# PimDeWitte/pde-engine

Hardware: AMD Instinct MI355X
Metric: validated candidates/sec (force-free depth-4 batch, 64x64 grid + p*) (higher is better)
Workload: dtype f64; 1 GPU; force_free validated candidates (force_free_d4_validated.npz, 142004 programs) tiled+shuffled(seed 0) to 2097152/GPU; 64x64 grid + ref point; problem=force_free, candidates_per_gpu=2097152, points_per_candidate=4097, full_grid=True, parallelism=shard1

## Files before the change

pde-engine_amd/csrc/pdeval.hip:

```cpp
#include <dlfcn.h>
#include <hip/hip_runtime.h>
#include <rccl/rccl.h>

#include <algorithm>
#include <cmath>
#include <cstdlib>
#include <cstdio>
#include <cstring>
#include <map>
#include <string>
#include <vector>

#include "../../include/pdeval.h"
#include "pdeval_kernels.h"
#include "pdeval_point.h"
#include "pdeval_tier2.h"
#include "pdeval_launch.h"
#include "pdeval_foliation.h"

using namespace pd;

#define PD_VERSION "pdeval 0.2 gfx950"

enum {
    L_DEFER = 0,
    L_CPLX = 1,
    L_DEFER2 = 2,
    L_ESC = 3,
    L_ESC_DEEP = 4,
    L_ESC_C = 5,
    L_CPLX_DEEP = 6,
    L_ESC_DEEP2 = 7,
    L_PDEEP = 8,
    L_DD = 9,
    L_DDC = 10,
    L_DD8 = 11,
    L_ESC_C_DEEP = 12,
    L_SLOW = 13,
    L_SLOW2 = 14,
    L_SLOW_C = 15,
    L_DDL = 16,
    L_DDLC = 17,
    L_DDL8 = 18,
    PD_N_LISTS = 19
};
enum { Q_PASS2 = 0, Q_CPLX, Q_T2, Q_T2_3, Q_T2_8, Q_T2_C, Q_T2_C8, Q_N };
#ifndef PD_LIST_QUEUE
#define PD_LIST_QUEUE 0
#endif
#ifndef PD_LIST_PARTS
#define PD_LIST_PARTS 1
#endif
constexpr int PD_COUNT_WORDS = PD_N_LISTS + 1 + Q_N;

namespace {
struct Grid {
    double x_lo, x_hi, nx, y_lo, y_hi, ny, x_ph, y_ph;
};
}

struct pdeval_ctx {
    int device = 0;
    int problem = 0;
    int n_ref = 0, n_pts = 0;
    int fp_pts[PDEVAL_FP_N] = {0, 0, 0, 0};
    hipStream_t stream = nullptr;
    hipStream_t side = nullptr;
    hipEvent_t ev_fork = nullptr, ev_join = nullptr;
    bool dd_early = true;
    int list_queue = PD_LIST_QUEUE;
    int list_parts = PD_LIST_PARTS;
    uint8_t* d_ddps = nullptr;
    double* d_dd_res = nullptr;
    double* d_dd_q = nullptr;
    bool dd_spec = true;
    double ref_x[4] = {0, 0, 0, 0}, ref_y[4] = {0, 0, 0, 0};
    dd ref_xd[4] = {}, ref_yd[4] = {};
    dd kc_ref[16] = {};
    int nx = 0, ny = 0;
    double* d_gx = nullptr;
    double* d_gy = nullptr;
    double* d_kc = nullptr;
    double* d_ptab = nullptr;
    Grid grid{};
    bool grid_default = true;
    pdeval_kerr_constants kconst{};
    PrmTab<double> prm_pt{}, prm_grid{};
    PrmTab<dd> prm_pt_dd{}, prm_grid_dd{};
    double ct_x[8] = {}, ct_y[8] = {};
    int n_ct = 0;
    int64_t cap = 0;
    int64_t* d_list[PD_N_LISTS] = {};
    int32_t* d_counts = nullptr;
    uint8_t* d_pstate = nullptr;
    int32_t* d_dec = nullptr;
    int64_t dec_cap = 0;
    bool hoist = true;
    bool hoist_sub = true;
    double* d_hoist = nullptr;
    uint32_t* d_hoist_own = nullptr;
    bool hoist_slots = true;
    int32_t* d_hseg = nullptr;
// ... 262 lines not shown
    }
    c->nx = nx;
    c->ny = ny;
    c->n_pts = c->n_ref + nx * ny;
    const int G = nx * ny;
    c->fp_pts[0] = 0;
    for (int f = 1; f < PDEVAL_FP_N; ++f) c->fp_pts[f] = c->n_ref + (int)((int64_t)G * f / PDEVAL_FP_N) + 7 % G;
    auto fail = [&](const char* what, hipError_t e) {
        g_err = std::string(what) + ": " + hipGetErrorString(e);
        pdeval_destroy(c);
        return PDEVAL_ERR_HIP;
    };
    hipError_t e;
    if ((e = hipSetDevice(device_id)) != hipSuccess) return fail("hipSetDevice", e);
    if (const char* v = getenv("PDEVAL_SORT")) c->sort = atoi(v) != 0;
    if (const char* v = getenv("PDEVAL_LEAN_CPLX")) c->lean_cplx = atoi(v) != 0;
    if (const char* v = getenv("PDEVAL_GRAPH")) c->use_graph = atoi(v) != 0;
    if (const char* v = getenv("PDEVAL_DD_EARLY")) c->dd_early = atoi(v) != 0;
    if (const char* v = getenv("PDEVAL_DD_SPEC")) c->dd_spec = atoi(v) != 0;
    if (const char* v = getenv("PDEVAL_LIST_QUEUE")) c->list_queue = std::max(0, atoi(v));
    if (const char* v = getenv("PDEVAL_LIST_PARTS")) c->list_parts = std::min(16, std::max(1, atoi(v)));
    if (const char* v = getenv("PDEVAL_HOIST")) c->hoist = atoi(v) != 0;
    if (const char* v = getenv("PDEVAL_HOIST_SUB")) c->hoist_sub = atoi(v) != 0;
    if (const char* v = getenv("PDEVAL_HOIST_SLOTS")) c->hoist_slots = atoi(v) != 0;
    if (const char* v = getenv("PDEVAL_TIER2_MASK")) c->tier2_mask = atoi(v) != 0;
    if (const char* v = getenv("PDEVAL_DEEP_PARTS")) c->deep_parts = atoi(v) > 1 ? PD_DEEP_PARTS : 1;
    if ((e = hipStreamCreateWithFlags(&c->stream, hipStreamNonBlocking)) != hipSuccess)
        return fail("hipStreamCreate", e);
    if ((e = hipStreamCreateWithFlags(&c->side, hipStreamNonBlocking)) != hipSuccess)
        return fail("hipStreamCreate", e);
    if ((e = hipEventCreateWithFlags(&c->ev_fork, hipEventDisableTiming)) != hipSuccess ||
        (e = hipEventCreateWithFlags(&c->ev_join, hipEventDisableTiming)) != hipSuccess)
        return fail("hipEventCreate", e);
    if ((e = hipMalloc(&c->d_gx, 2 * nx * sizeof(double))) != hipSuccess) return fail("hipMalloc", e);
    if ((e = hipMalloc(&c->d_gy, ny * sizeof(double))) != hipSuccess) return fail("hipMalloc", e);
    if (problem_id == PDEVAL_PROBLEM_KERR &&
        (e = hipMalloc(&c->d_kc, 8 * (size_t)c->n_pts * sizeof(double))) != hipSuccess)
        return fail("hipMalloc", e);
    if (problem_id == PDEVAL_PROBLEM_KERR) pdeval_default_kerr_constants(&c->kconst);
    if (int rc = build_points(c)) {
        g_err = c->err;
        pdeval_destroy(c);
        return rc;
    }
    if ((e = hipMalloc(&c->d_counts, PD_COUNT_WORDS * sizeof(int32_t))) != hipSuccess) return fail("hipMalloc", e);
    *out = c;
    return PDEVAL_OK;
}

extern "C" int pdeval_destroy(pdeval_ctx* c) {
    if (!c) return PDEVAL_ERR_ARG;
    (void)hipSetDevice(c->device);
    if (c->stream) (void)hipStreamSynchronize(c->stream);
    if (c->side) (void)hipStreamSynchronize(c->side);
    if (c->comm) pdeval_comm_destroy(c);
    for (int64_t* l : c->d_list)
        if (l) (void)hipFree(l);
    if (c->d_pstate) (void)hipFree(c->d_pstate);
    if (c->d_ddps) (void)hipFree(c->d_ddps);
    if (c->d_dd_res) (void)hipFree(c->d_dd_res);
    if (c->d_dd_q) (void)hipFree(c->d_dd_q);
    if (c->d_dec) (void)hipFree(c->d_dec);
    if (c->d_hoist) (void)hipFree(c->d_hoist);
    if (c->d_hoist_own) (void)hipFree(c->d_hoist_own);
    if (c->d_hseg) (void)hipFree(c->d_hseg);
    if (c->d_fmask) (void)hipFree(c->d_fmask);
    if (c->d_fsum) (void)hipFree(c->d_fsum);
    if (c->d_status) (void)hipFree(c->d_status);
    if (c->d_noise) (void)hipFree(c->d_noise);
    if (c->d_t2acc) (void)hipFree(c->d_t2acc);
    if (c->d_skeys) (void)hipFree(c->d_skeys);
    if (c->d_sidx) (void)hipFree(c->d_sidx);
    if (c->d_stemp) (void)hipFree(c->d_stemp);
    for (void* p : {(void*)c->d_gx, (void*)c->d_gy, (void*)c->d_kc, (void*)c->d_ptab,
                    (void*)c->d_counts, (void*)c->d_ops, (void*)c->d_off, (void*)c->d_outbuf})
        if (p) (void)hipFree(p);
    for (auto& g : c->graphs)
        if (g.second.exec) (void)hipGraphExecDestroy(g.second.exec);
    if (c->h_stage) (void)hipHostFree(c->h_stage);
    if (c->h_errw) (void)hipHostFree(c->h_errw);
    for (hipEvent_t& e : c->ev)
        if (e) (void)hipEventDestroy(e);
    if (c->ev_fork) (void)hipEventDestroy(c->ev_fork);
    if (c->ev_join) (void)hipEventDestroy(c->ev_join);
    if (c->side) (void)hipStreamDestroy(c->side);
    if (c->stream) (void)hipStreamDestroy(c->stream);
    delete c;
    return PDEVAL_OK;
}

extern "C" const char* pdeval_last_error(pdeval_ctx* c) { return c ? c->err.c_str() : g_err.c_str(); }
extern "C" int pdeval_n_ref_points(pdeval_ctx* c) { return c ? c->n_ref : -1; }
extern "C" int pdeval_n_points(pdeval_ctx* c) { return c ? c->n_pts : -1; }
extern "C" const char* pdeval_version(void) { return PD_VERSION; }

extern "C" int pdeval_default_params(int problem_id, pdeval_params* p) {
    if (!p) return PDEVAL_ERR_ARG;
    p->tau_point = 1e-10;
    p->tau_grid = 1e-7;
    p->kerr_abs_tol = 1e-10;
    p->full_grid = 1;
    p->max_bad = 0;
    p->strict_symbolic = 1;
    p->reserved = 0;
    p->noise_kappa = 16.0;
    p->point_abs_tol = 1e-20;
    p->res_rel_acc = 1e-11;
    p->omega2 = 0.0;
    p->omega2_lo = 0.0;
    (void)problem_id;
    return PDEVAL_OK;
}

static int op_has_imm(uint32_t op) {
    return op == PDOP_PUSH_C || op == PDOP_ADDC || op == PDOP_MULC || op == PDOP_RDIVC || op == PDOP_POW;
}
static int op_words(int32_t w) {
// ... 234 lines not shown
    if (c->d_hseg) (void)hipFree(c->d_hseg);
    c->d_hseg = nullptr;
    if (c->hoist) {
        const int K = c->problem == PDEVAL_PROBLEM_FORCE_FREE ? 4 : 2;
        if (c->hoist_slots && !c->d_hoist) {
            HIPCHK(c, hipMalloc(&c->d_hoist, (size_t)8 * pd::kHoistPool * pd::hoist_stride(K) * sizeof(double)));
            HIPCHK(c, hipMalloc(&c->d_hoist_own, (size_t)8 * pd::kHoistPool * sizeof(uint32_t)));
            HIPCHK(c, hipMemset(c->d_hoist_own, 0, (size_t)8 * pd::kHoistPool * sizeof(uint32_t)));
        } else if (!c->hoist_slots) {
            if (c->d_hoist) (void)hipFree(c->d_hoist);
            c->d_hoist = nullptr;
            HIPCHK(c, hipMalloc(&c->d_hoist, (size_t)std::max<int64_t>(cap, 8 * pd::kHoistPool) * pd::hoist_stride(K) * sizeof(double)));
        }
        HIPCHK(c, hipMalloc(&c->d_hseg, (size_t)cap * 4 * sizeof(int32_t)));
    }
    if (c->d_fmask) (void)hipFree(c->d_fmask);
    c->d_fmask = nullptr;
    if (c->d_fsum) (void)hipFree(c->d_fsum);
    c->d_fsum = nullptr;
    if (c->tier2_mask) {
        HIPCHK(c, hipMalloc(&c->d_fmask, (size_t)cap * c->nx * (c->ny / 64) * sizeof(uint64_t)));
        HIPCHK(c, hipMalloc(&c->d_fsum, (size_t)cap * sizeof(uint64_t)));
    }
    if (c->d_status) (void)hipFree(c->d_status);
    c->d_status = nullptr;
    HIPCHK(c, hipMalloc(&c->d_status, cap));
    if (c->d_noise) (void)hipFree(c->d_noise);
    c->d_noise = nullptr;
    HIPCHK(c, hipMalloc(&c->d_noise, cap * 4 * sizeof(double)));
    if (c->d_t2acc) (void)hipFree(c->d_t2acc);
    c->d_t2acc = nullptr;
    HIPCHK(c, hipMalloc(&c->d_t2acc, cap * sizeof(T2Acc)));
    HIPCHK(c, hipMemset(c->d_t2acc, 0, cap * sizeof(T2Acc)));
    if (c->d_skeys) (void)hipFree(c->d_skeys);
    if (c->d_sidx) (void)hipFree(c->d_sidx);
    if (c->d_stemp) (void)hipFree(c->d_stemp);
    c->d_skeys = nullptr;
    c->d_sidx = nullptr;
    c->d_stemp = nullptr;
    HIPCHK(c, hipMalloc(&c->d_skeys, 2 * cap * sizeof(uint64_t)));
    HIPCHK(c, hipMalloc(&c->d_sidx, 2 * cap * sizeof(int32_t)));
    c->stemp_bytes = sort_temp_bytes(cap);
    HIPCHK(c, hipMalloc(&c->d_stemp, c->stemp_bytes ? c->stemp_bytes : 16));
    c->cap = cap;
    return PDEVAL_OK;
}

template <class T, int K, int MAXD> constexpr size_t stack_lds(int waves) {
    return (size_t)waves * (MAXD - 1) * ((K + 1) * (K + 2) / 2) * 64 * sizeof(T);
}

#ifndef PD_T2_PARTS
#define PD_T2_PARTS 4
#endif
#ifndef PD_T2_PARTS_C
#define PD_T2_PARTS_C 16
#endif
template <class T, int K, int MAXD> constexpr size_t tier2_lds() {
    return (size_t)(MAXD - 1) * ((K + 1) * (K + 2) / 2) * 64 * (sizeof(T) + sizeof(double));
}

#ifndef PD_DD_EARLY_MIN_N
#define PD_DD_EARLY_MIN_N 1024
#endif

__global__ __launch_bounds__(256) void sanitize_list_kernel(const int64_t* list, int32_t* count, int64_t cap,
// ... 118 lines not shown
        KernelArgs b = follow(L_PDEEP, -1, L_ESC);
        launch_point_list(PROB, 0, lgrid, s, b);
        HIPCHK(c, hipGetLastError());
    }
    if constexpr (FF) {
        KernelArgs b = follow(L_CPLX, -1, L_ESC_C);
        launch_point_list(PROB, 1, lgrid, s, b);
        HIPCHK(c, hipGetLastError());
    }
    auto dd_lists = [&](int l0, int lc, int l8) {
        KernelArgs b = a;
        b.defer_list = c->d_list[l0];
        b.defer_count = cnt + l0;
        b.cplx_list = c->d_list[lc];
        b.cplx_count = cnt + lc;
        b.esc_list = c->d_list[l8];
        b.esc_count = cnt + l8;
        return b;
    };
    const unsigned cgrid = (unsigned)((n + 255) / 256);
    const bool early = c->dd_early && n >= PD_DD_EARLY_MIN_N;
    a.dd_spec = early && c->dd_spec ? 1 : 0;
    if (early) {
        hipLaunchKernelGGL((dd_collect_kernel<PROB, DD_EARLY>), dim3(cgrid), dim3(256), 0, s, dd_lists(L_DD, L_DDC, L_DD8));
        HIPCHK(c, hipGetLastError());
        HIPCHK(c, hipEventRecord(c->ev_fork, s));
        HIPCHK(c, hipStreamWaitEvent(c->side, c->ev_fork, 0));
        launch_dd_point(PROB, 0, lgrid, c->side, follow(L_DD, -1, L_ESC), true);
        if (dmax > 2) launch_dd_point(PROB, 1, lgrid, c->side, follow(L_DD8, -1, L_ESC), true);
        if constexpr (FF) launch_dd_point(PROB, 2, lgrid, c->side, follow(L_DDC, -1, L_ESC), true);
        HIPCHK(c, hipGetLastError());
        HIPCHK(c, hipEventRecord(c->ev_join, c->side));
    }
    mark(2);
    launch_decode(PROB, n, s, a);
    HIPCHK(c, hipGetLastError());
    launch_grid(PROB, n, s, a, c->d_list[L_SLOW], cnt + L_SLOW);
    HIPCHK(c, hipGetLastError());
    hipLaunchKernelGGL((validate_kernel<PROB, double, 2, true>), dim3((unsigned)std::min<int64_t>(blocks, 256)),
                       dim3(64), (stack_lds<double, K, 2>(1)), s, follow(L_SLOW, L_DEFER, L_ESC));
    HIPCHK(c, hipGetLastError());
    mark(3);
    if (dmax > 2) {
        hipLaunchKernelGGL(sanitize_list_kernel, dim3(64), dim3(256), 0, s, c->d_list[L_DEFER], cnt + L_DEFER, c->cap, n,
                           a.errw, (uint32_t)ERRW_GRID_LIST);
        launch_grid_list(PROB, pgrid, s, queue(follow(L_DEFER, L_DEFER2, L_ESC), Q_PASS2), c->d_list[L_SLOW2],
                         cnt + L_SLOW2, lparts);
        HIPCHK(c, hipGetLastError());
        hipLaunchKernelGGL((validate_kernel<PROB, double, 3, true>), dim3((unsigned)std::min<int64_t>(blocks, 256)),
                           dim3(64), (stack_lds<double, K, 3>(1)), s, follow(L_SLOW2, L_DEFER2, L_ESC));
        HIPCHK(c, hipGetLastError());
    }
    mark(4);
    if (dmax > 3) {
        if (c->deep_parts > 1)
            hipLaunchKernelGGL((validate_kernel<PROB, double, PDEVAL_MAX_STACK, true, PD_DEEP_PARTS>),
                               dim3((unsigned)std::min<int64_t>(4 * blocks, 1024)), dim3(64),
                               (stack_lds<double, K, PDEVAL_MAX_STACK>(1)), s, follow(L_DEFER2, -1, L_ESC));
        else
            hipLaunchKernelGGL((validate_kernel<PROB, double, PDEVAL_MAX_STACK, true>),
                               dim3((unsigned)std::min<int64_t>(4 * blocks, 1024)), dim3(64),
                               (stack_lds<double, K, PDEVAL_MAX_STACK>(1)), s, follow(L_DEFER2, -1, L_ESC));
        HIPCHK(c, hipGetLastError());
    }
    if constexpr (FF) {
        mark(5);
        if (c->lean_cplx) {
            hipLaunchKernelGGL(sanitize_list_kernel, dim3(64), dim3(256), 0, s, c->d_list[L_CPLX], cnt + L_CPLX, c->cap,
                               n, a.errw, (uint32_t)ERRW_CPLX);
            launch_grid_cplx(pgrid, s, queue(follow(L_CPLX, L_CPLX_DEEP, L_ESC_C), Q_CPLX), c->d_list[L_SLOW_C],
                             cnt + L_SLOW_C, lparts);
            HIPCHK(c, hipGetLastError());
            hipLaunchKernelGGL((validate_kernel<PROB, cplx, 2, true>), dim3((unsigned)std::min<int64_t>(blocks, 256)),
                               dim3(64), (stack_lds<cplx, K, 2>(1)), s, follow(L_SLOW_C, L_CPLX_DEEP, L_ESC_C));
        } else {
            hipLaunchKernelGGL((validate_kernel<PROB, cplx, 2, true>), dim3(pgrid), dim3(64),
                               (stack_lds<cplx, K, 2>(1)), s, follow(L_CPLX, L_CPLX_DEEP, L_ESC_C));
        }
        HIPCHK(c, hipGetLastError());
        mark(6);
        if (dmax > 2) {
            if (c->deep_parts > 1)
                hipLaunchKernelGGL((validate_kernel<PROB, cplx, PDEVAL_MAX_STACK, true, PD_DEEP_PARTS>),
                                   dim3((unsigned)std::min<int64_t>(4 * blocks, 512)), dim3(64),
                                   (stack_lds<cplx, K, PDEVAL_MAX_STACK>(1)), s, follow(L_CPLX_DEEP, -1, L_ESC_C));
            else
                hipLaunchKernelGGL((validate_kernel<PROB, cplx, PDEVAL_MAX_STACK, true>),
                                   dim3((unsigned)std::min<int64_t>(4 * blocks, 512)), dim3(64),
                                   (stack_lds<cplx, K, PDEVAL_MAX_STACK>(1)), s, follow(L_CPLX_DEEP, -1, L_ESC_C));
            HIPCHK(c, hipGetLastError());
        }
    } else {
        mark(5);
        mark(6);
    }
    KernelArgs t = queue(follow(L_ESC, L_ESC_DEEP, L_ESC), Q_T2);
    mark(7);
    hipLaunchKernelGGL((tier2_kernel<PROB, double, 2, false, PD_T2_PARTS>), dim3((unsigned)std::min<int64_t>(n * PD_T2_PARTS, 8192)),
                       dim3(64), (tier2_lds<double, K, 2>()), s, t);
    HIPCHK(c, hipGetLastError());
    mark(8);
    if (dmax > 2) {
        hipLaunchKernelGGL((tier2_kernel<PROB, double, 3, false, PD_T2_PARTS>), dim3((unsigned)std::min<int64_t>(n * PD_T2_PARTS, 4096)),
                           dim3(64), (tier2_lds<double, K, 3>()), s, queue(follow(L_ESC_DEEP, L_ESC_DEEP2, L_ESC), Q_T2_3));
        HIPCHK(c, hipGetLastError());
    }
    mark(9);
    if (dmax > 3) {
        hipLaunchKernelGGL((tier2_kernel<PROB, double, PDEVAL_MAX_STACK>), dim3((unsigned)std::min<int64_t>(n, 512)),
                           dim3(64), (tier2_lds<double, K, PDEVAL_MAX_STACK>()), s, queue(follow(L_ESC_DEEP2, -1, L_ESC), Q_T2_8));
        HIPCHK(c, hipGetLastError());
    }
    if constexpr (FF) {
        mark(10);
        hipLaunchKernelGGL((tier2_kernel<PROB, cplx, 4, false, PD_T2_PARTS_C>),
                           dim3((unsigned)std::min<int64_t>(n * PD_T2_PARTS_C, 4096)), dim3(64),
                           (tier2_lds<cplx, K, 4>()), s, queue(follow(L_ESC_C, L_ESC_C_DEEP, L_ESC_C), Q_T2_C));
        HIPCHK(c, hipGetLastError());
        if (dmax > 4) {
            hipLaunchKernelGGL((tier2_kernel<PROB, cplx, PDEVAL_MAX_STACK, true>), dim3((unsigned)std::min<int64_t>(n, 256)),
                               dim3(64), 0, s, queue(follow(L_ESC_C_DEEP, -1, L_ESC_C), Q_T2_C8));
            HIPCHK(c, hipGetLastError());
        }
    } else {
        mark(10);
    }
    mark(11);
    if (early) {
        HIPCHK(c, hipStreamWaitEvent(s, c->ev_join, 0));
        hipLaunchKernelGGL((dd_collect_kernel<PROB, DD_LATE>), dim3(cgrid), dim3(256), 0, s, dd_lists(L_DDL, L_DDLC, L_DDL8));
        HIPCHK(c, hipGetLastError());
        launch_dd_point(PROB, 0, lgrid, s, follow(L_DDL, -1, L_ESC));
        if (dmax > 2) launch_dd_point(PROB, 1, lgrid, s, follow(L_DDL8, -1, L_ESC));
        if constexpr (FF) launch_dd_point(PROB, 2, lgrid, s, follow(L_DDLC, -1, L_ESC));
        HIPCHK(c, hipGetLastError());
        launch_dd_apply(PROB, (unsigned)std::min<int64_t>(cgrid, 1024), s, dd_lists(L_DD, L_DDC, L_DD8));
        HIPCHK(c, hipGetLastError());
    } else {
        hipLaunchKernelGGL((dd_collect_kernel<PROB, DD_ALL>), dim3(cgrid), dim3(256), 0, s, dd_lists(L_DD, L_DDC, L_DD8));
        HIPCHK(c, hipGetLastError());
        launch_dd_point(PROB, 0, lgrid, s, follow(L_DD, -1, L_ESC));
        if (dmax > 2) launch_dd_point(PROB, 1, lgrid, s, follow(L_DD8, -1, L_ESC));
        if constexpr (FF) launch_dd_point(PROB, 2, lgrid, s, follow(L_DDC, -1, L_ESC));
        HIPCHK(c, hipGetLastError());
    }
    mark(PDEVAL_N_PASSES);
    c->ev_recorded = c->timing ? 1 : 0;
    return PDEVAL_OK;
}

static int check_errw(pdeval_ctx* c, uint32_t w, const char* path, int64_t n, int captured);

static int validate_device(pdeval_ctx* c, const int32_t* d_ops, int64_t n_words, const int64_t* d_offsets,
                           int64_t n, const pdeval_params* params, const pdeval_outputs* d_out, void* stream,
                           int zero_bits, int dmax) {
    if (!c || !d_out || n < 0 || (n > 0 && (!d_ops || !d_offsets)) || n_words < 0) {
        if (c) c->err = "pdeval_validate_device: bad argument";
        return PDEVAL_ERR_ARG;
// ... 69 lines not shown
        d->q_grid = (double*)p; p += 8 * n;
        d->res_ref = (double*)p; p += 8 * n * c->n_ref;
        d->fingerprint = (double*)p; p += 8 * n * PDEVAL_FP_N;
        d->n_bad = (int32_t*)p; p += 4 * n;
        d->n_nonfinite = (int32_t*)p;
    }
    return need;
}

static int validate_small(pdeval_ctx* c, const int32_t* ops, int64_t n_words, const int64_t* offsets, int64_t n,
                          const pdeval_params* params, pdeval_outputs* out, int dmax) {
    if (n_words > kSmallWords) return kGraphFallback;
    if (c->hcap_words < kSmallWords || c->hcap_n < PD_GRAPH_MAX_N + 1) {
        ++c->buf_epoch;
        const int64_t w = std::max<int64_t>(kSmallWords, c->hcap_words);
        const int64_t m = std::max<int64_t>(PD_GRAPH_MAX_N + 1, c->hcap_n);
        if (c->d_ops) (void)hipFree(c->d_ops);
        if (c->d_off) (void)hipFree(c->d_off);
        c->d_ops = nullptr;
        c->d_off = nullptr;
        c->hcap_words = c->hcap_n = 0;
        HIPCHK(c, hipMalloc(&c->d_ops, w * sizeof(int32_t)));
        HIPCHK(c, hipMalloc(&c->d_off, m * sizeof(int64_t)));
        c->hcap_words = w;
        c->hcap_n = m;
    }
    const int64_t need_max = outbuf_layout(c, PD_GRAPH_MAX_N, nullptr);
    if (c->outbuf_bytes < need_max) {
        ++c->buf_epoch;
        if (c->d_outbuf) (void)hipFree(c->d_outbuf);
        c->d_outbuf = nullptr;
        c->outbuf_bytes = 0;
        HIPCHK(c, hipMalloc(&c->d_outbuf, need_max));
        c->outbuf_bytes = need_max;
    }
    int rc = ensure_scratch(c, n);
    if (rc) return rc;
    rc = ensure_dec(c, c->hcap_words);
    if (rc) return rc;
    const size_t in_bytes = kSmallWords * 4 + (PD_GRAPH_MAX_N + 1) * 8;
    if (!c->h_stage) {
        HIPCHK(c, hipHostMalloc((void**)&c->h_stage, in_bytes + need_max + 16, hipHostMallocDefault));
        c->h_stage_bytes = in_bytes + need_max + 16;
    }
    pdeval_params prm;
    if (params) prm = *params;
    else pdeval_default_params(c->problem, &prm);
    dmax = dmax <= 2 ? 2 : dmax <= 4 ? dmax : PDEVAL_MAX_STACK;
    uint64_t key = 1469598103934665603ull;
    auto mix = [&](const void* p, size_t len) {
        const uint8_t* b = (const uint8_t*)p;
        for (size_t i = 0; i < len; ++i) key = (key ^ b[i]) * 1099511628211ull;
    };
    mix(&n, sizeof(n));
    mix(&dmax, sizeof(dmax));
    mix(&prm, sizeof(prm));
    pdeval_outputs d{};
    const int64_t need = outbuf_layout(c, n, &d);
    hipStream_t s = c->stream;
    auto it = c->graphs.find(key);
    if (it != c->graphs.end() && it->second.epoch != c->buf_epoch) {
        (void)hipGraphExecDestroy(it->second.exec);
        c->graphs.erase(it);
        it = c->graphs.end();
    }
    int fresh = 0;
// ... 80 lines not shown
        }
        dmax = std::max(dmax, d);
    }
    HIPCHK(c, hipSetDevice(c->device));
    if (n <= PD_GRAPH_MAX_N && c->use_graph && !c->timing) {
        const int rc = validate_small(c, ops, n_words, offsets, n, params, out, dmax);
        if (rc != kGraphFallback) return rc;
    }
    if (n_words > c->hcap_words) {
        ++c->buf_epoch;
        if (c->d_ops) (void)hipFree(c->d_ops);
        c->d_ops = nullptr;
        c->hcap_words = 0;
        HIPCHK(c, hipMalloc(&c->d_ops, n_words * sizeof(int32_t)));
        c->hcap_words = n_words;
    }
    if (n + 1 > c->hcap_n) {
        ++c->buf_epoch;
        if (c->d_off) (void)hipFree(c->d_off);
        c->d_off = nullptr;
        c->hcap_n = 0;
        HIPCHK(c, hipMalloc(&c->d_off, (n + 1) * sizeof(int64_t)));
        c->hcap_n = n + 1;
    }
    const int64_t nb = ((n + 31) / 32) * 4;
    const int64_t sz_bits = (nb + 15) / 16 * 16, sz_st = (n + 15) / 16 * 16;
    const int64_t need = sz_bits + sz_st + 8 * n * (3 + c->n_ref + PDEVAL_FP_N) + 8 * n * 2;
    if (need > c->outbuf_bytes) {
        ++c->buf_epoch;
        if (c->d_outbuf) (void)hipFree(c->d_outbuf);
        c->d_outbuf = nullptr;
        c->outbuf_bytes = 0;
        HIPCHK(c, hipMalloc(&c->d_outbuf, need));
        c->outbuf_bytes = need;
    }
    uint8_t* p = c->d_outbuf;
    pdeval_outputs d{};
    d.verdict_bits = p; p += sz_bits;
    d.status = p; p += sz_st;
    d.q_ref = (double*)p; p += 8 * n;
    d.q_grid = (double*)p; p += 8 * n;
    d.res_ref = (double*)p; p += 8 * n * c->n_ref;
    d.fingerprint = (double*)p; p += 8 * n * PDEVAL_FP_N;
    d.n_bad = (int32_t*)p; p += 4 * n;
    d.n_nonfinite = (int32_t*)p; p += 4 * n;
    hipStream_t s = c->stream;
    HIPCHK(c, hipMemcpyAsync(c->d_ops, ops, n_words * sizeof(int32_t), hipMemcpyHostToDevice, s));
    HIPCHK(c, hipMemcpyAsync(c->d_off, offsets, (n + 1) * sizeof(int64_t), hipMemcpyHostToDevice, s));
    int rc = validate_device(c, c->d_ops, n_words, c->d_off, n, params, &d, s, 1, dmax);
    if (rc) return rc;
    auto dl = [&](void* h, const void* dv, size_t bytes) -> int {
        if (h) HIPCHK(c, hipMemcpyAsync(h, dv, bytes, hipMemcpyDeviceToHost, s));
        return PDEVAL_OK;
    };
    if ((rc = dl(out->verdict_bits, d.verdict_bits, (n + 7) / 8))) return rc;
    if ((rc = dl(out->status, d.status, n))) return rc;
    if ((rc = dl(out->q_ref, d.q_ref, 8 * n))) return rc;
    if ((rc = dl(out->q_grid, d.q_grid, 8 * n))) return rc;
    if ((rc = dl(out->res_ref, d.res_ref, 8 * n * c->n_ref))) return rc;
    if ((rc = dl(out->fingerprint, d.fingerprint, 8 * n * PDEVAL_FP_N))) return rc;
    if ((rc = dl(out->n_bad, d.n_bad, 4 * n))) return rc;
    if ((rc = dl(out->n_nonfinite, d.n_nonfinite, 4 * n))) return rc;
    uint32_t* herr = reinterpret_cast<uint32_t*>(c->h_errw);
    if (!herr) {
        HIPCHK(c, hipHostMalloc((void**)&c->h_errw, 16, hipHostMallocDefault));
        herr = reinterpret_cast<uint32_t*>(c->h_errw);
// ... 5 lines not shown

extern "C" int pdeval_set_timing(pdeval_ctx* c, int enable) {
    if (!c) return PDEVAL_ERR_ARG;
    HIPCHK(c, hipSetDevice(c->device));
    if (enable && !c->ev[0])
        for (hipEvent_t& e : c->ev) HIPCHK(c, hipEventCreate(&e));
    c->timing = enable != 0;
    c->ev_recorded = 0;
    return PDEVAL_OK;
}

extern "C" int pdeval_pass_times(pdeval_ctx* c, float* ms, int max_passes, const char** names) {
    if (!c || !ms || max_passes < 0) return PDEVAL_ERR_ARG;
    if (!c->ev_recorded) {
        c->err = "pdeval_pass_times: no timed call (pdeval_set_timing(ctx, 1) first)";
        return PDEVAL_ERR_ARG;
    }
    HIPCHK(c, hipSetDevice(c->device));
    HIPCHK(c, hipEventSynchronize(c->ev[PDEVAL_N_PASSES]));
    const int n = max_passes < PDEVAL_N_PASSES ? max_passes : PDEVAL_N_PASSES;
    for (int k = 0; k < n; ++k) {
        HIPCHK(c, hipEventElapsedTime(&ms[k], c->ev[k], c->ev[k + 1]));
        if (names) names[k] = kPassNames[k];
    }
    return PDEVAL_OK;
}

extern "C" int pdeval_pass_counts(pdeval_ctx* c, int64_t* counts, int max_counts) {
    if (!c || !counts || max_counts < 0) return PDEVAL_ERR_ARG;
    HIPCHK(c, hipSetDevice(c->device));
    int32_t h[PD_N_LISTS] = {0};
    HIPCHK(c, hipDeviceSynchronize());
    HIPCHK(c, hipMemcpy(h, c->d_counts, sizeof(h), hipMemcpyDeviceToHost));
    for (int k = 0; k < max_counts && k < PD_N_LISTS; ++k) counts[k] = h[k];
    return PDEVAL_OK;
}

extern "C" int pdeval_eval_points(pdeval_ctx* c, const int32_t* prog, int64_t n_words, const double* xs,
                                  const double* ys, int n_pts, int tier2, double* out, double* jets) {
    if (!c || !prog || !xs || !ys || !out || n_pts <= 0 || n_pts > (1 << 20)) return PDEVAL_ERR_ARG;
    const int d = pdeval_program_depth(prog, n_words);
    if (d < 0 || d > PDEVAL_MAX_STACK) {
        c->err = "pdeval_eval_points: malformed program";
        return PDEVAL_ERR_PROGRAM;
    }
    if (c->problem == PDEVAL_PROBLEM_KERR) {
        c->err = "pdeval_eval_points: force-free only";
        return PDEVAL_ERR_ARG;
    }
    HIPCHK(c, hipSetDevice(c->device));
    int32_t* d_prog = nullptr;
    double *d_x = nullptr, *d_y = nullptr, *d_out = nullptr, *d_jets = nullptr;
    const size_t jet_bytes = (size_t)n_pts * 2 * 15 * sizeof(double);
    auto cleanup = [&]() {
        for (void* q : {(void*)d_prog, (void*)d_x, (void*)d_y, (void*)d_out, (void*)d_jets})
            if (q) (void)hipFree(q);
    };
    hipError_t e = hipSuccess;
    if ((e = hipMalloc(&d_prog, n_words * 4)) == hipSuccess && (e = hipMalloc(&d_x, n_pts * 8)) == hipSuccess &&
        (e = hipMalloc(&d_y, n_pts * 8)) == hipSuccess && (e = hipMalloc(&d_out, n_pts * 32)) == hipSuccess &&
        (e = hipMemcpy(d_prog, prog, n_words * 4, hipMemcpyHostToDevice)) == hipSuccess &&
        (e = hipMemcpy(d_x, xs, n_pts * 8, hipMemcpyHostToDevice)) == hipSuccess &&
        (e = hipMemcpy(d_y, ys, n_pts * 8, hipMemcpyHostToDevice)) == hipSuccess &&
        (!jets || (e = hipMalloc(&d_jets, jet_bytes)) == hipSuccess)) {
        constexpr int K = 4, MAXD = PDEVAL_MAX_STACK;
        hipLaunchKernelGGL((eval_points_kernel<PDEVAL_PROBLEM_FORCE_FREE, MAXD>), dim3((n_pts + 63) / 64), dim3(64),
// ... 153 lines not shown
```

pde-engine_amd/csrc/pdeval_grid.h:

```cpp
#pragma once

#include "pdeval_kernels.h"

namespace pd {

#ifndef PD_LEAN_RSLOT
#define PD_LEAN_RSLOT 1
#endif

constexpr uint64_t op_bit(int op) { return 1ull << op; }
constexpr int PTAB_N = 17;
constexpr uint64_t kImmMask = op_bit(PDOP_PUSH_C) | op_bit(PDOP_ADDC) | op_bit(PDOP_MULC) |
                              op_bit(PDOP_RDIVC) | op_bit(PDOP_POW);
constexpr uint64_t kPushMask = op_bit(PDOP_PUSH_X) | op_bit(PDOP_PUSH_Y) | op_bit(PDOP_PUSH_C) |
                               op_bit(PDOP_PUSH_P);
constexpr uint64_t kBinMask = op_bit(PDOP_ADD) | op_bit(PDOP_SUB) | op_bit(PDOP_RSUB) |
                              op_bit(PDOP_MUL) | op_bit(PDOP_DIV) | op_bit(PDOP_RDIV);
constexpr uint64_t kUnaryMask =
    op_bit(PDOP_ADDC) | op_bit(PDOP_MULC) | op_bit(PDOP_RDIVC) | op_bit(PDOP_NEG) |
    op_bit(PDOP_ADD_X) | op_bit(PDOP_ADD_Y) | op_bit(PDOP_SUB_X) | op_bit(PDOP_SUB_Y) |
    op_bit(PDOP_MUL_X) | op_bit(PDOP_MUL_Y) | op_bit(PDOP_DIV_X) | op_bit(PDOP_DIV_Y) |
    op_bit(PDOP_POWN) | op_bit(PDOP_POW) | op_bit(PDOP_EXP) | op_bit(PDOP_LOG) | op_bit(PDOP_ABS) |
    op_bit(PDOP_SQRT) | op_bit(PDOP_ADD_P) | op_bit(PDOP_SUB_P) | op_bit(PDOP_MUL_P) |
    op_bit(PDOP_DIV_P) | op_bit(PDOP_RDIV_P);
// ... 243 lines not shown
        last = pc;
        pc += len;
    }
    ok = ok && d == 1 && last >= 0;
    if (ok) dec[last] |= (int32_t)(1u << 20);
    uint32_t hp = 0u;
    if (PD_HOIST && ok && hoist_last >= 0 && hoist_heavy) {
        const uint32_t at = (uint32_t)hoist_last + (((uint32_t)dec[hoist_last] >> DEC_DIST) & DEC_DIST_MAX);
        if (at < (uint32_t)plen && at < (1u << 14)) hp = at;
    }
    dec[0] = ok ? (int32_t)(((uint32_t)dmax << 8) | (sg[1] < 0 ? 1u << 16 : 0u) | (hp << 17) |
                            (hp && hoist_y ? 1u << 31 : 0u)) : (int32_t)0xff;
    if (a.hseg) {
        int best = -1;
        const bool cplx = (hdr & PDEVAL_FLAG_COMPLEX) || (a.pstate && (a.pstate[cand] & P0_CPLX));
        if (hoist_sub<PROB>() && ok && !cplx)
            for (int k = 0; k < nseg; ++k)
                if (sg_hs[k] >= (int)hp && (!sg_y[k] || (PROB != PDEVAL_PROBLEM_FORCE_FREE && a.ny == 64)) &&
                    (best < 0 || sg_nh[k] > sg_nh[best]))
                    best = k;
        int32_t* hs = a.hseg + 4 * cand;
        if (best >= 0) {
            const int at = sg_hs[best], to = sg_he[best];
            hs[0] = dec[at];
            hs[1] = at;
            hs[2] = to;
            hs[3] = sg_y[best] ? 1 : 0;
            dec[at] = (int32_t)(DOP_PUSH_H | (DG_PUSH << 17) | ((uint32_t)(to - at) << DEC_DIST) |
                                (1u << (DEC_ONEHOT + DG_PUSH)));
        } else {
            hs[1] = 0;
        }
    }
}

template <int K> constexpr size_t ptab_doubles(int nx, int ny) { return (size_t)PTAB_N * (K + 1) * (size_t)(nx + ny); }
template <int K>
__global__ __launch_bounds__(256) void ptab_kernel(const double* gx, const double* gy, int nx, int ny, double* tab) {
    const int64_t t = (int64_t)blockIdx.x * blockDim.x + threadIdx.x;
    const int64_t nxt = (int64_t)PTAB_N * nx;
    double pk[K + 1];
    if (t < nxt) {
        const int n = (int)(t / nx), i = (int)(t % nx);
        JetOps<double, K>::pcoefs(gx[i], n, pk);
#pragma unroll
        for (int k = 0; k <= K; ++k) tab[((size_t)n * nx + i) * (K + 1) + k] = pk[k];
    } else if (t < nxt + (int64_t)PTAB_N * ny) {
        const int64_t u = t - nxt;
        const int n = (int)(u / ny), j = (int)(u % ny);
        JetOps<double, K>::pcoefs(gy[j], n, pk);
        double* ty = tab + nxt * (K + 1);
#pragma unroll
        for (int k = 0; k <= K; ++k) ty[((size_t)n * (K + 1) + k) * ny + j] = pk[k];
    }
}
#ifndef PD_PTAB
#define PD_PTAB 2
#endif
#ifndef PD_PTAB_KERR
#define PD_PTAB_KERR 0
#endif
template <int W> struct PowTab {
    const double* px[W];
    const double* py;
    int sx, sy, ny;
};
// ... 482 lines not shown
        if (got < 0) {
            if (a.errw) atomicOr(a.errw, (uint32_t)ERRW_HOIST);
            got = (int)(base + home);
        }
    }
    return (int64_t)__builtin_amdgcn_readfirstlane(got);
}
__device__ __forceinline__ void hoist_release(const KernelArgs& a, int64_t slot, int lane, bool split) {
    if (!PD_HOIST_SLOTS || split || !a.hoist_own || a.hoist_pool <= 0 || slot < 0) return;
#ifndef PD_HOST_SIM
    asm volatile("s_waitcnt vmcnt(0)" ::: "memory");
#endif
    if (lane == 0) __hip_atomic_store(a.hoist_own + slot, 0u, __ATOMIC_RELAXED, __HIP_MEMORY_SCOPE_AGENT);
}

template <int PROB, int MAXD, class T = double, bool ROT = false>
__device__ __forceinline__ void grid_body(const KernelArgs& a, int64_t cand, int lane, T* stk,
                                          int64_t* slow_list, int32_t* slow_count, int part = 0,
                                          int parts = 1) {
    constexpr int K = grid_k<PROB>();
    constexpr int W = grid_w<PROB, MAXD>();
    constexpr bool CX = Real<T>::cplx_pass;
    using L = Lean<T, K, W, MAXD>;
    using J = typename L::J;
    const int64_t beg = a.offsets[cand], end = a.offsets[cand + 1];
    const bool in_bounds = beg >= 0 && end > beg && end <= a.n_words && end - beg < (1 << 24);
    const int32_t* prog = a.ops + (in_bounds ? beg : 0);
    const uint32_t hdr = in_bounds ? rd_word(prog) : 0xffu;
    const uint8_t ps = (uint8_t)__builtin_amdgcn_readfirstlane((int)a.pstate[cand]);
    if (!CX && (ps & P0_CPLX)) return;
    if ((ps & 3) == P0_REJECT && !a.prm.full_grid) return;
    bool slow = !in_bounds || (hdr & 0xffu) != 0u || (ps & 3) == P0_NONE || (!CX && (hdr & PDEVAL_FLAG_COMPLEX));
    if (!slow && (int)((hdr >> 8) & 0xffu) > MAXD) {
        if (lane == 0 && part == 0) list_append(a.defer_list, a.defer_count, a.list_capacity, cand);
        return;
    }
    uint32_t u_sgn = 0u;
    int hoist = 0;
    bool hy = false;
    int h_at = 0, h_to = 0;
    bool h_y = false;
    uint32_t h_w0 = 0u;
    if (!slow) {
        const uint32_t dh = rd_word(a.dec + beg);
        slow = (dh & 0xffu) != 0u || (int)((dh >> 8) & 0xffu) > MAXD;
        u_sgn = (dh & 0x10000u) << 15;
        if (!CX && hoist_sub<PROB>() && a.hseg && !slow) {
            const int32_t* hs = a.hseg + 4 * cand;
            h_at = __builtin_amdgcn_readfirstlane(hs[1]);
            if (h_at) {
                h_w0 = (uint32_t)__builtin_amdgcn_readfirstlane(hs[0]);
                h_to = __builtin_amdgcn_readfirstlane(hs[2]);
                h_y = __builtin_amdgcn_readfirstlane(hs[3]) != 0;
            }
        }
        if (!CX && PD_HOIST && a.hoist && parts == 1) {
            hoist = (int)((dh >> 17) & 0x3fffu);
            hy = (dh >> 31) != 0u;
            if (hy && (PROB == PDEVAL_PROBLEM_FORCE_FREE || a.ny != 64)) hoist = 0;
            if (PROB == PDEVAL_PROBLEM_FORCE_FREE) hy = false;
        }
    }
    if (slow) {
        if (lane == 0 && part == 0) list_append(slow_list, slow_count, a.list_capacity, cand);
        return;
    }
    const int per_row = a.ny >> 6;
// ... 249 lines not shown
```

Before: 13.33 million candidates/s.

## Overlap deferred and complex list passes with main grid pass on a second stream

```diff
diff --git a/pde-engine_amd/csrc/pdeval.hip b/pde-engine_amd/csrc/pdeval.hip
--- a/pde-engine_amd/csrc/pdeval.hip
+++ b/pde-engine_amd/csrc/pdeval.hip
@@ -42,7 +42,11 @@
     L_DDL = 16,
     L_DDLC = 17,
     L_DDL8 = 18,
-    PD_N_LISTS = 19
+    L_DEFER_L = 19,
+    L_DEFER2_L = 20,
+    L_CPLX_L = 21,
+    L_CPLX_DEEP_L = 22,
+    PD_N_LISTS = 23
 };
 enum { Q_PASS2 = 0, Q_CPLX, Q_T2, Q_T2_3, Q_T2_8, Q_T2_C, Q_T2_C8, Q_N };
 #ifndef PD_LIST_QUEUE
@@ -68,6 +72,11 @@
     hipStream_t side = nullptr;
     hipEvent_t ev_fork = nullptr, ev_join = nullptr;
     bool dd_early = true;
+    hipStream_t lists = nullptr;
+    hipEvent_t ev_lfork = nullptr, ev_ljoin = nullptr, ev_t2fork = nullptr, ev_t2join = nullptr;
+    bool list_overlap = true;
+    int list_order = 0;
+    T2Acc* d_t2acc_l = nullptr;
     int list_queue = PD_LIST_QUEUE;
     int list_parts = PD_LIST_PARTS;
     uint8_t* d_ddps = nullptr;
@@ -396,6 +405,15 @@
     if ((e = hipEventCreateWithFlags(&c->ev_fork, hipEventDisableTiming)) != hipSuccess ||
         (e = hipEventCreateWithFlags(&c->ev_join, hipEventDisableTiming)) != hipSuccess)
         return fail("hipEventCreate", e);
+    if (const char* v = getenv("PDEVAL_LIST_OVERLAP")) c->list_overlap = atoi(v) != 0;
+    if (const char* v = getenv("PDEVAL_LIST_ORDER")) c->list_order = atoi(v) != 0;
+    if (c->list_overlap) {
+        if ((e = hipStreamCreateWithFlags(&c->lists, hipStreamNonBlocking)) != hipSuccess)
+            return fail("hipStreamCreate", e);
+        for (hipEvent_t* ev : {&c->ev_lfork, &c->ev_ljoin, &c->ev_t2fork, &c->ev_t2join})
+            if ((e = hipEventCreateWithFlags(ev, hipEventDisableTiming)) != hipSuccess)
+                return fail("hipEventCreate", e);
+    }
     if ((e = hipMalloc(&c->d_gx, 2 * nx * sizeof(double))) != hipSuccess) return fail("hipMalloc", e);
     if ((e = hipMalloc(&c->d_gy, ny * sizeof(double))) != hipSuccess) return fail("hipMalloc", e);
     if (problem_id == PDEVAL_PROBLEM_KERR &&
@@ -417,6 +435,7 @@
     (void)hipSetDevice(c->device);
     if (c->stream) (void)hipStreamSynchronize(c->stream);
     if (c->side) (void)hipStreamSynchronize(c->side);
+    if (c->lists) (void)hipStreamSynchronize(c->lists);
     if (c->comm) pdeval_comm_destroy(c);
     for (int64_t* l : c->d_list)
         if (l) (void)hipFree(l);
@@ -433,6 +452,7 @@
     if (c->d_status) (void)hipFree(c->d_status);
     if (c->d_noise) (void)hipFree(c->d_noise);
     if (c->d_t2acc) (void)hipFree(c->d_t2acc);
+    if (c->d_t2acc_l) (void)hipFree(c->d_t2acc_l);
     if (c->d_skeys) (void)hipFree(c->d_skeys);
     if (c->d_sidx) (void)hipFree(c->d_sidx);
     if (c->d_stemp) (void)hipFree(c->d_stemp);
@@ -447,6 +467,9 @@
         if (e) (void)hipEventDestroy(e);
     if (c->ev_fork) (void)hipEventDestroy(c->ev_fork);
     if (c->ev_join) (void)hipEventDestroy(c->ev_join);
+    for (hipEvent_t ev : {c->ev_lfork, c->ev_ljoin, c->ev_t2fork, c->ev_t2join})
+        if (ev) (void)hipEventDestroy(ev);
+    if (c->lists) (void)hipStreamDestroy(c->lists);
     if (c->side) (void)hipStreamDestroy(c->side);
     if (c->stream) (void)hipStreamDestroy(c->stream);
     delete c;
@@ -747,6 +770,12 @@
     c->d_t2acc = nullptr;
     HIPCHK(c, hipMalloc(&c->d_t2acc, cap * sizeof(T2Acc)));
     HIPCHK(c, hipMemset(c->d_t2acc, 0, cap * sizeof(T2Acc)));
+    if (c->d_t2acc_l) (void)hipFree(c->d_t2acc_l);
+    c->d_t2acc_l = nullptr;
+    if (c->list_overlap) {
+        HIPCHK(c, hipMalloc(&c->d_t2acc_l, cap * sizeof(T2Acc)));
+        HIPCHK(c, hipMemset(c->d_t2acc_l, 0, cap * sizeof(T2Acc)));
+    }
     if (c->d_skeys) (void)hipFree(c->d_skeys);
     if (c->d_sidx) (void)hipFree(c->d_sidx);
     if (c->d_stemp) (void)hipFree(c->d_stemp);
@@ -931,69 +960,145 @@
         HIPCHK(c, hipGetLastError());
         HIPCHK(c, hipEventRecord(c->ev_join, c->side));
     }
-    mark(2);
-    launch_decode(PROB, n, s, a);
-    HIPCHK(c, hipGetLastError());
-    launch_grid(PROB, n, s, a, c->d_list[L_SLOW], cnt + L_SLOW);
-    HIPCHK(c, hipGetLastError());
-    hipLaunchKernelGGL((validate_kernel<PROB, double, 2, true>), dim3((unsigned)std::min<int64_t>(blocks, 256)),
-                       dim3(64), (stack_lds<double, K, 2>(1)), s, follow(L_SLOW, L_DEFER, L_ESC));
-    HIPCHK(c, hipGetLastError());
-    mark(3);
-    if (dmax > 2) {
-        hipLaunchKernelGGL(sanitize_list_kernel, dim3(64), dim3(256), 0, s, c->d_list[L_DEFER], cnt + L_DEFER, c->cap, n,
-                           a.errw, (uint32_t)ERRW_GRID_LIST);
-        launch_grid_list(PROB, pgrid, s, queue(follow(L_DEFER, L_DEFER2, L_ESC), Q_PASS2), c->d_list[L_SLOW2],
-                         cnt + L_SLOW2, lparts);
-        HIPCHK(c, hipGetLastError());
+    const bool lov = c->list_overlap && c->lists && !c->timing && n >= PD_DD_EARLY_MIN_N;
+    hipStream_t const ls = lov ? c->lists : s;
+    auto on = [&](KernelArgs b, int lc, bool list_stream) {
+        b.cplx_list = FF ? c->d_list[lc] : nullptr;
+        b.cplx_count = cnt + lc;
+        if (lov && list_stream) b.t2acc = c->d_t2acc_l;
+        return b;
+    };
+    auto generic3 = [&](hipStream_t st, const KernelArgs& b) {
         hipLaunchKernelGGL((validate_kernel<PROB, double, 3, true>), dim3((unsigned)std::min<int64_t>(blocks, 256)),
-                           dim3(64), (stack_lds<double, K, 3>(1)), s, follow(L_SLOW2, L_DEFER2, L_ESC));
-        HIPCHK(c, hipGetLastError());
-    }
-    mark(4);
-    if (dmax > 3) {
+                           dim3(64), (stack_lds<double, K, 3>(1)), st, b);
+    };
+    auto deep8 = [&](hipStream_t st, const KernelArgs& b) {
         if (c->deep_parts > 1)
             hipLaunchKernelGGL((validate_kernel<PROB, double, PDEVAL_MAX_STACK, true, PD_DEEP_PARTS>),
                                dim3((unsigned)std::min<int64_t>(4 * blocks, 1024)), dim3(64),
-                               (stack_lds<double, K, PDEVAL_MAX_STACK>(1)), s, follow(L_DEFER2, -1, L_ESC));
+                               (stack_lds<double, K, PDEVAL_MAX_STACK>(1)), st, b);
         else
             hipLaunchKernelGGL((validate_kernel<PROB, double, PDEVAL_MAX_STACK, true>),
                                dim3((unsigned)std::min<int64_t>(4 * blocks, 1024)), dim3(64),
-                               (stack_lds<double, K, PDEVAL_MAX_STACK>(1)), s, follow(L_DEFER2, -1, L_ESC));
-        HIPCHK(c, hipGetLastError());
-    }
-    if constexpr (FF) {
+                               (stack_lds<double, K, PDEVAL_MAX_STACK>(1)), st, b);
+    };
+    auto generic_c2 = [&](hipStream_t st, unsigned grid, const KernelArgs& b) {
+        hipLaunchKernelGGL((validate_kernel<PROB, cplx, 2, true>), dim3(grid), dim3(64), (stack_lds<cplx, K, 2>(1)), st, b);
+    };
+    auto deep_c8 = [&](hipStream_t st, const KernelArgs& b) {
+        if (c->deep_parts > 1)
+            hipLaunchKernelGGL((validate_kernel<PROB, cplx, PDEVAL_MAX_STACK, true, PD_DEEP_PARTS>),
+                               dim3((unsigned)std::min<int64_t>(4 * blocks, 512)), dim3(64),
+                               (stack_lds<cplx, K, PDEVAL_MAX_STACK>(1)), st, b);
+        else
+            hipLaunchKernelGGL((validate_kernel<PROB, cplx, PDEVAL_MAX_STACK, true>),
+                               dim3((unsigned)std::min<int64_t>(4 * blocks, 512)), dim3(64),
+                               (stack_lds<cplx, K, PDEVAL_MAX_STACK>(1)), st, b);
+    };
+    auto real_lists = [&](int lc) -> int {
+        mark(3);
+        if (dmax > 2) {
+            hipLaunchKernelGGL(sanitize_list_kernel, dim3(64), dim3(256), 0, ls, c->d_list[L_DEFER], cnt + L_DEFER, c->cap, n,
+                               a.errw, (uint32_t)ERRW_GRID_LIST);
+            launch_grid_list(PROB, pgrid, ls, queue(on(follow(L_DEFER, L_DEFER2, L_ESC), lc, true), Q_PASS2),
+                             c->d_list[L_SLOW2], cnt + L_SLOW2, lparts);
+            HIPCHK(c, hipGetLastError());
+            generic3(ls, on(follow(L_SLOW2, L_DEFER2, L_ESC), lc, true));
+            HIPCHK(c, hipGetLastError());
+        }
+        mark(4);
+        if (dmax > 3) {
+            deep8(ls, on(follow(L_DEFER2, -1, L_ESC), lc, true));
+            HIPCHK(c, hipGetLastError());
+        }
+        return PDEVAL_OK;
+    };
+    auto cplx_lists = [&]() -> int {
         mark(5);
         if (c->lean_cplx) {
-            hipLaunchKernelGGL(sanitize_list_kernel, dim3(64), dim3(256), 0, s, c->d_list[L_CPLX], cnt + L_CPLX, c->cap,
+            hipLaunchKernelGGL(sanitize_list_kernel, dim3(64), dim3(256), 0, ls, c->d_list[L_CPLX], cnt + L_CPLX, c->cap,
                                n, a.errw, (uint32_t)ERRW_CPLX);
-            launch_grid_cplx(pgrid, s, queue(follow(L_CPLX, L_CPLX_DEEP, L_ESC_C), Q_CPLX), c->d_list[L_SLOW_C],
-                             cnt + L_SLOW_C, lparts);
+            launch_grid_cplx(pgrid, ls, queue(on(follow(L_CPLX, L_CPLX_DEEP, L_ESC_C), L_CPLX, true), Q_CPLX),
+                             c->d_list[L_SLOW_C], cnt + L_SLOW_C, lparts);
             HIPCHK(c, hipGetLastError());
-            hipLaunchKernelGGL((validate_kernel<PROB, cplx, 2, true>), dim3((unsigned)std::min<int64_t>(blocks, 256)),
-                               dim3(64), (stack_lds<cplx, K, 2>(1)), s, follow(L_SLOW_C, L_CPLX_DEEP, L_ESC_C));
+            generic_c2(ls, (unsigned)std::min<int64_t>(blocks, 256), on(follow(L_SLOW_C, L_CPLX_DEEP, L_ESC_C), L_CPLX, true));
         } else {
-            hipLaunchKernelGGL((validate_kernel<PROB, cplx, 2, true>), dim3(pgrid), dim3(64),
-                               (stack_lds<cplx, K, 2>(1)), s, follow(L_CPLX, L_CPLX_DEEP, L_ESC_C));
+            generic_c2(ls, pgrid, on(follow(L_CPLX, L_CPLX_DEEP, L_ESC_C), L_CPLX, true));
         }
         HIPCHK(c, hipGetLastError());
         mark(6);
         if (dmax > 2) {
-            if (c->deep_parts > 1)
-                hipLaunchKernelGGL((validate_kernel<PROB, cplx, PDEVAL_MAX_STACK, true, PD_DEEP_PARTS>),
-                                   dim3((unsigned)std::min<int64_t>(4 * blocks, 512)), dim3(64),
-                                   (stack_lds<cplx, K, PDEVAL_MAX_STACK>(1)), s, follow(L_CPLX_DEEP, -1, L_ESC_C));
-            else
-                hipLaunchKernelGGL((validate_kernel<PROB, cplx, PDEVAL_MAX_STACK, true>),
-                                   dim3((unsigned)std::min<int64_t>(4 * blocks, 512)), dim3(64),
-                                   (stack_lds<cplx, K, PDEVAL_MAX_STACK>(1)), s, follow(L_CPLX_DEEP, -1, L_ESC_C));
+            deep_c8(ls, on(follow(L_CPLX_DEEP, -1, L_ESC_C), L_CPLX, true));
             HIPCHK(c, hipGetLastError());
         }
+        return PDEVAL_OK;
+    };
+    mark(2);
+    {
+        KernelArgs da = a;
+        if (!lov) da.defer_list = nullptr;
+        launch_decode(PROB, n, s, da);
+        HIPCHK(c, hipGetLastError());
+    }
+    if (lov) {
+        HIPCHK(c, hipEventRecord(c->ev_lfork, s));
+        HIPCHK(c, hipStreamWaitEvent(ls, c->ev_lfork, 0));
+        KernelArgs pa = a;
+        pa.defer_list = nullptr;
+        launch_grid(PROB, n, s, pa, c->d_list[L_SLOW], cnt + L_SLOW);
+        HIPCHK(c, hipGetLastError());
+        hipLaunchKernelGGL((validate_kernel<PROB, double, 2, true>), dim3((unsigned)std::min<int64_t>(blocks, 256)),
+                           dim3(64), (stack_lds<double, K, 2>(1)), s, on(follow(L_SLOW, L_DEFER_L, L_ESC), L_CPLX_L, false));
+        HIPCHK(c, hipGetLastError());
+        if (c->list_order == 0) {
+            if (int rc = real_lists(L_CPLX)) return rc;
+        }
+        if constexpr (FF) {
+            if (int rc = cplx_lists()) return rc;
+        }
+        if (c->list_order != 0) {
+            if (int rc = real_lists(L_CPLX_L)) return rc;
+        }
+        HIPCHK(c, hipEventRecord(c->ev_ljoin, ls));
+        HIPCHK(c, hipStreamWaitEvent(s, c->ev_ljoin, 0));
+        if (dmax > 2) generic3(s, on(follow(L_DEFER_L, L_DEFER2_L, L_ESC), L_CPLX_L, false));
+        if (dmax > 3) deep8(s, on(follow(L_DEFER2_L, -1, L_ESC), L_CPLX_L, false));
+        if constexpr (FF) {
+            generic_c2(s, (unsigned)std::min<int64_t>(blocks, 256), follow(L_CPLX_L, L_CPLX_DEEP_L, L_ESC_C));
+            if (dmax > 2) deep_c8(s, follow(L_CPLX_DEEP_L, -1, L_ESC_C));
+        }
+        HIPCHK(c, hipGetLastError());
     } else {
-        mark(5);
-        mark(6);
+        launch_grid(PROB, n, s, a, c->d_list[L_SLOW], cnt + L_SLOW);
+        HIPCHK(c, hipGetLastError());
+        hipLaunchKernelGGL((validate_kernel<PROB, double, 2, true>), dim3((unsigned)std::min<int64_t>(blocks, 256)),
+                           dim3(64), (stack_lds<double, K, 2>(1)), s, follow(L_SLOW, L_DEFER, L_ESC));
+        HIPCHK(c, hipGetLastError());
+        if (int rc = real_lists(L_CPLX)) return rc;
+        if constexpr (FF) {
+            if (int rc = cplx_lists()) return rc;
+        } else {
+            mark(5);
+            mark(6);
+        }
     }
     KernelArgs t = queue(follow(L_ESC, L_ESC_DEEP, L_ESC), Q_T2);
+    auto tier2_cplx = [&]() -> int {
+        hipLaunchKernelGGL((tier2_kernel<PROB, cplx, 4, false, PD_T2_PARTS_C>),
+                           dim3((unsigned)std::min<int64_t>(n * PD_T2_PARTS_C, 4096)), dim3(64),
+                           (tier2_lds<cplx, K, 4>()), ls, queue(on(follow(L_ESC_C, L_ESC_C_DEEP, L_ESC_C), L_CPLX, true), Q_T2_C));
+        HIPCHK(c, hipGetLastError());
+        if (dmax > 4) {
+            hipLaunchKernelGGL((tier2_kernel<PROB, cplx, PDEVAL_MAX_STACK, true>), dim3((unsigned)std::min<int64_t>(n, 256)),
+                               dim3(64), 0, ls, queue(on(follow(L_ESC_C_DEEP, -1, L_ESC_C), L_CPLX, true), Q_T2_C8));
+            HIPCHK(c, hipGetLastError());
+        }
+        return PDEVAL_OK;
+    };
+    if (FF && lov) {
+        HIPCHK(c, hipEventRecord(c->ev_t2fork, s));
+        HIPCHK(c, hipStreamWaitEvent(ls, c->ev_t2fork, 0));
+    }
     mark(7);
     hipLaunchKernelGGL((tier2_kernel<PROB, double, 2, false, PD_T2_PARTS>), dim3((unsigned)std::min<int64_t>(n * PD_T2_PARTS, 8192)),
                        dim3(64), (tier2_lds<double, K, 2>()), s, t);
@@ -1010,19 +1115,13 @@
                            dim3(64), (tier2_lds<double, K, PDEVAL_MAX_STACK>()), s, queue(follow(L_ESC_DEEP2, -1, L_ESC), Q_T2_8));
         HIPCHK(c, hipGetLastError());
     }
+    mark(10);
     if constexpr (FF) {
-        mark(10);
-        hipLaunchKernelGGL((tier2_kernel<PROB, cplx, 4, false, PD_T2_PARTS_C>),
-                           dim3((unsigned)std::min<int64_t>(n * PD_T2_PARTS_C, 4096)), dim3(64),
-                           (tier2_lds<cplx, K, 4>()), s, queue(follow(L_ESC_C, L_ESC_C_DEEP, L_ESC_C), Q_T2_C));
-        HIPCHK(c, hipGetLastError());
-        if (dmax > 4) {
-            hipLaunchKernelGGL((tier2_kernel<PROB, cplx, PDEVAL_MAX_STACK, true>), dim3((unsigned)std::min<int64_t>(n, 256)),
-                               dim3(64), 0, s, queue(follow(L_ESC_C_DEEP, -1, L_ESC_C), Q_T2_C8));
-            HIPCHK(c, hipGetLastError());
-        }
-    } else {
-        mark(10);
+        if (int rc = tier2_cplx()) return rc;
+        if (lov) {
+            HIPCHK(c, hipEventRecord(c->ev_t2join, ls));
+            HIPCHK(c, hipStreamWaitEvent(s, c->ev_t2join, 0));
+        }
     }
     mark(11);
     if (early) {
@@ -1158,6 +1257,7 @@
         c->d_outbuf = nullptr;
         c->outbuf_bytes = 0;
         HIPCHK(c, hipMalloc(&c->d_outbuf, need_max));
+        HIPCHK(c, hipMemsetAsync(c->d_outbuf, 0, need_max, c->stream));
         c->outbuf_bytes = need_max;
     }
     int rc = ensure_scratch(c, n);
@@ -1304,6 +1404,7 @@
         c->d_outbuf = nullptr;
         c->outbuf_bytes = 0;
         HIPCHK(c, hipMalloc(&c->d_outbuf, need));
+        HIPCHK(c, hipMemsetAsync(c->d_outbuf, 0, need, c->stream));
         c->outbuf_bytes = need;
     }
     uint8_t* p = c->d_outbuf;
@@ -1375,6 +1476,10 @@
     int32_t h[PD_N_LISTS] = {0};
     HIPCHK(c, hipDeviceSynchronize());
     HIPCHK(c, hipMemcpy(h, c->d_counts, sizeof(h), hipMemcpyDeviceToHost));
+    h[L_DEFER] += h[L_DEFER_L];
+    h[L_DEFER2] += h[L_DEFER2_L];
+    h[L_CPLX] += h[L_CPLX_L];
+    h[L_CPLX_DEEP] += h[L_CPLX_DEEP_L];
     for (int k = 0; k < max_counts && k < PD_N_LISTS; ++k) counts[k] = h[k];
     return PDEVAL_OK;
 }
diff --git a/pde-engine_amd/csrc/pdeval_grid.h b/pde-engine_amd/csrc/pdeval_grid.h
--- a/pde-engine_amd/csrc/pdeval_grid.h
+++ b/pde-engine_amd/csrc/pdeval_grid.h
@@ -299,6 +299,13 @@
             hs[1] = 0;
         }
     }
+    if (a.defer_list && a.pstate) {
+        const uint8_t ps = a.pstate[cand];
+        const bool skip = (ps & P0_CPLX) || ((ps & 3) == P0_REJECT && !a.prm.full_grid);
+        const bool slow = (hdr & 0xffu) != 0u || (ps & 3) == P0_NONE || (hdr & PDEVAL_FLAG_COMPLEX);
+        if (!skip && !slow && (int)((hdr >> 8) & 0xffu) > 2)
+            list_append(a.defer_list, a.defer_count, a.list_capacity, cand);
+    }
 }
 
 template <int K> constexpr size_t ptab_doubles(int nx, int ny) { return (size_t)PTAB_N * (K + 1) * (size_t)(nx + ny); }
@@ -847,7 +854,7 @@
     if ((ps & 3) == P0_REJECT && !a.prm.full_grid) return;
     bool slow = !in_bounds || (hdr & 0xffu) != 0u || (ps & 3) == P0_NONE || (!CX && (hdr & PDEVAL_FLAG_COMPLEX));
     if (!slow && (int)((hdr >> 8) & 0xffu) > MAXD) {
-        if (lane == 0 && part == 0) list_append(a.defer_list, a.defer_count, a.list_capacity, cand);
+        if (lane == 0 && part == 0 && a.defer_list) list_append(a.defer_list, a.defer_count, a.list_capacity, cand);
         return;
     }
     uint32_t u_sgn = 0u;
```

Measured after the change: 13.43 million candidates/s, median of 6. No clear change (+0.7%).
